# erlgo/openair4G

Measured on AMD Instinct MI355X. Metric: DL subframes/sec (20 MHz, 2x2, 64-QAM), higher is better.
Workload: dtype int16; 1 GPU; dlsim 20 MHz 2x2 TM3 (LARGE_CDD) 64-QAM MCS19x2CW, 2x14 IDFT-2048; config_id=C3, global_batch=8192, subframe_index=7, full_grid=False, parallelism=subframe-sharded x1

## Files before the change

### openair4g_amd/csrc/oai4g_encode.hip

```cpp
#include "oai4g_internal.h"

struct rsc_tables_t {
  uint8_t next[8][16];
  uint8_t par[8][16];
  uint8_t apow[8][8];
  uint32_t hz;
  uint32_t zs[8];
  uint32_t fm[3];
};

static constexpr uint8_t rsc_step_c(uint8_t u, uint8_t s, uint8_t *out)
{
  *out = (uint8_t)((u ^ (s >> 2) ^ (s >> 1)) & 1);
  return (uint8_t)((((u << 2) ^ (s >> 1)) ^ ((s >> 1) << 2) ^ (s << 2)) & 7);
}

static constexpr rsc_tables_t make_rsc_tables()
{
  rsc_tables_t t{};
  for (int s = 0; s < 8; s++)
    for (int nib = 0; nib < 16; nib++) {
      uint8_t st = (uint8_t)s, p = 0;
      for (int b = 0; b < 4; b++) {
        uint8_t o = 0;
// ... 90 lines not shown
typedef const __attribute__((address_space(1))) uint32_t gu32_t;

[[maybe_unused]] static __device__ __forceinline__ void gold_generate(uint32_t *gold, uint32_t nwords, uint32_t c_init,
                                                     const uint32_t *gx1, const uint32_t *gx2j)
{
  const uint32_t l = threadIdx.x, w0 = OAI4G_GOLD_STRIDE * l;
  if (l >= OAI4G_GOLD_LANES || w0 >= nwords) return;
  const uint32_t x2i = c_init ^ ((c_init ^ (c_init >> 1) ^ (c_init >> 2) ^ (c_init >> 3)) << 31);
  gu32_t *col = (gu32_t *)(gx2j + l);
  uint32_t cv[32];
#pragma unroll
  for (int b = 0; b < 32; b++) cv[b] = col[OAI4G_GOLD_LANES * b];
  uint32_t x2 = 0;
#pragma unroll
  for (int b = 0; b < 32; b++) x2 ^= cv[b] & (0u - ((x2i >> b) & 1u));
  uint32_t x1 = *(gu32_t *)(gx1 + l);
  const uint32_t wend = min(w0 + OAI4G_GOLD_STRIDE, nwords);
  gold[w0] = x1 ^ x2;
  for (uint32_t w = w0 + 1; w < wend; w++) {
    gold_step(x1, x2);
    gold[w] = x1 ^ x2;
  }
}

static __device__ __forceinline__ uint32_t crc_step(uint32_t reg, uint32_t byte, const uint32_t *tab)
{
  return ((reg << 8) & 0xffffffu) ^ tab[((reg >> 16) ^ byte) & 0xffu];
}

static __device__ __forceinline__ uint32_t crc_mul_tab(uint32_t a, const uint32_t *t )
{
  return t[a & 15u] ^ t[16 + ((a >> 4) & 15u)] ^ t[32 + ((a >> 8) & 15u)] ^ t[48 + ((a >> 12) & 15u)] ^
         t[64 + ((a >> 16) & 15u)] ^ t[80 + ((a >> 20) & 15u)];
}

static __device__ __forceinline__ uint32_t crc_chunk(const uint8_t *buf, uint32_t nbytes, uint32_t per, uint32_t lane,
                                                     uint32_t nl, const uint32_t *tab)
{
  const int vstart = (int)(lane * per) - (int)(per * nl - nbytes);
  uint32_t reg = 0;
  for (uint32_t i = 0; i < per; i += 4) {
    uint32_t b[4];
#pragma unroll
    for (int q = 0; q < 4; q++) {
      const int idx = vstart + (int)i + q;
      b[q] = idx >= 0 ? (uint32_t)buf[idx] : 0u;
    }
#pragma unroll
    for (int q = 0; q < 4; q++) reg = crc_step(reg, b[q], tab);
  }
  return reg;
}

static __device__ __forceinline__ uint32_t crc_chunk_w(const uint32_t *base32, uint32_t start, uint32_t nbytes,
                                                       uint32_t per, uint32_t lane, uint32_t nl, const uint32_t *tab8)
{
  const int vstart = (int)(lane * per) - (int)(per * nl - nbytes);
  uint32_t reg = 0;
  for (uint32_t i = 0; i < per; i += 4) {
    const int o = vstart + (int)i;
    const uint32_t a = start + (uint32_t)(o > 0 ? o : 0), wi = a >> 2;
    uint32_t w = __builtin_amdgcn_alignbit(base32[wi + 1], base32[wi], (a & 3u) * 8u);
    if (o < 0) w = o <= -4 ? 0u : w << (8 * (uint32_t)(-o));
    reg = (reg << 8) ^ tab8[(reg >> 24) ^ (w & 0xffu)];
    reg = (reg << 8) ^ tab8[(reg >> 24) ^ ((w >> 8) & 0xffu)];
    reg = (reg << 8) ^ tab8[(reg >> 24) ^ ((w >> 16) & 0xffu)];
    reg = (reg << 8) ^ tab8[(reg >> 24) ^ (w >> 24)];
  }
  return reg >> 8;
}

static __device__ __forceinline__ void crc_chunk_w2r(const uint32_t *base32, uint32_t start, uint32_t nbytes,
                                                     uint32_t per, uint32_t pos, uint32_t nl, const uint8_t *r2a,
                                                     const uint8_t *r2b, uint32_t &ra, uint32_t &rb)
{
  const int vstart = (int)(pos * per) - (int)(per * nl - nbytes);
  uint32_t a = 0, b = 0;
  for (uint32_t i = 0; i < per; i += 4) {
    const int o = vstart + (int)i;
    const uint32_t ad = start + (uint32_t)(o > 0 ? o : 0), wi = ad >> 2;
    uint32_t w = __builtin_amdgcn_alignbit(base32[wi + 1], base32[wi], (ad & 3u) * 8u);
    if (o < 0) w = o <= -4 ? 0u : w << (8 * (uint32_t)(-o));
    const uint32_t wr = __builtin_bitreverse32(w);
    const uint32_t x[4] = {wr >> 22, wr >> 14, wr >> 6, wr << 2};
#pragma unroll
    for (int q = 0; q < 4; q++) {
      a = (a >> 8) ^ *(const uint32_t *)(r2a + ((a ^ x[q]) & 0x3fcu));
      b = (b >> 8) ^ *(const uint32_t *)(r2b + ((b ^ x[q]) & 0x3fcu));
    }
  }
  ra = __builtin_bitreverse32(a >> 2) >> 8;
  rb = __builtin_bitreverse32(b >> 2) >> 8;
}

static __device__ __forceinline__ void crc_group_tree2(uint32_t &ra, uint32_t &rb, uint32_t pos, uint32_t lpb,
                                                       const uint32_t (*ma)[8][96], const uint32_t (*mb)[8][96])
{
  const uint32_t j0 = 7 - (pos & 7), j1 = (lpb >> 3) - 1 - (pos >> 3);
  ra = crc_mul_tab(ra, ma[0][j0]);
  rb = crc_mul_tab(rb, mb[0][j0]);
#pragma unroll
  for (int m = 1; m < 8; m <<= 1) {
    ra ^= __shfl_xor(ra, m, 64);
    rb ^= __shfl_xor(rb, m, 64);
  }
  ra = crc_mul_tab(ra, ma[1][j1]);
  rb = crc_mul_tab(rb, mb[1][j1]);
  for (uint32_t m = 8; m < lpb; m <<= 1) {
    ra ^= __shfl_xor(ra, (int)m, 64);
    rb ^= __shfl_xor(rb, (int)m, 64);
  }
}

[[maybe_unused]] static __device__ __forceinline__ uint32_t crc_wave_tree(uint32_t reg, const uint32_t *mul)
{
  const uint32_t lane = threadIdx.x & 63;
  for (int d = 0; d < 6; d++) {
    uint32_t other = __shfl_down(reg, 1u << d, 64);
    if ((lane & ((2u << d) - 1u)) == 0) reg = crc_mul_tab(reg, mul + d * 96) ^ other;
  }
  return reg;
}

static __device__ __forceinline__ uint32_t crc_wave_tree2(uint32_t reg, const uint32_t (*mul)[8][96])
{
  const uint32_t lane = threadIdx.x & 63;
  reg = crc_mul_tab(reg, mul[0][7 - (lane & 7)]);
  reg ^= __shfl_xor(reg, 1, 64);
  reg ^= __shfl_xor(reg, 2, 64);
  reg ^= __shfl_xor(reg, 4, 64);
  reg = crc_mul_tab(reg, mul[1][7 - (lane >> 3)]);
  reg ^= __shfl_xor(reg, 8, 64);
  reg ^= __shfl_xor(reg, 16, 64);
  reg ^= __shfl_xor(reg, 32, 64);
  return reg;
}

static __device__ __forceinline__ uint32_t crc_mulmod(uint32_t a, uint32_t b, uint32_t poly)
{
  uint32_t r = 0;
  for (int i = 23; i >= 0; i--) {
    r <<= 1;
    if (r & 0x1000000u) r ^= 0x1000000u | poly;
    if ((b >> i) & 1u) r ^= a;
  }
// ... 265 lines not shown
#pragma unroll
  for (int k = 0; k < 3; k++) {
    const uint32_t J = 4u >> k;
    const bool hi = (lane32 & J) != 0;
    t.rot[k] = hi ? J : 32u - J;
    t.mm[k] = hi ? ~M[k] : M[k];
  }
  return t;
}

template <int K = 0>
static __device__ __forceinline__ uint32_t transpose32_t(uint32_t x, const tp_lane_t &t)
{
  if constexpr (K == 5) {
    return x;
  } else if constexpr (K < 2) {
    const uint32_t p = xor_lane<(16u >> K)>(x);
    return transpose32_t<K + 1>(__builtin_amdgcn_perm(p, x, K == 0 ? t.sel16 : t.sel8), t);
  } else {
    const uint32_t p = xor_lane<(16u >> K)>(x);
    const uint32_t sh = __builtin_amdgcn_alignbit(p, p, t.rot[K - 2]);
    uint32_t r;
    asm("v_bitop3_b32 %0, %1, %2, %3 bitop3:0xe4" : "=v"(r) : "v"(x), "v"(sh), "v"(t.mm[K - 2]));
    return transpose32_t<K + 1>(r, t);
  }
}

static __device__ __forceinline__ void or_bits(uint32_t *w, uint32_t bit, uint32_t v)
{
  if (!v) return;
  const uint32_t wi = bit >> 5, sh = bit & 31u;
  atomicOr(&w[wi], v << sh);
  if (sh && (v >> (32 - sh))) atomicOr(&w[wi + 1], v >> (32 - sh));
}

static __device__ __forceinline__ void or_bits2(uint32_t *w, uint32_t bit, uint32_t v)
{
  const uint64_t s = (uint64_t)v << (bit & 31u);
  uint32_t *p = w + (bit >> 5);
  atomicOr(p, (uint32_t)s);
  atomicOr(p + 1, (uint32_t)(s >> 32));
}

template <bool DEBUG>
static __device__ void encode_codeword(const cfg_dev_t *__restrict__ c, uint32_t sf, uint32_t cwi,
                                       const uint8_t *__restrict__ payload, uint32_t *__restrict__ ebits,
                                       enc_debug_t dbg, uint32_t *lds_base, int stop_phase = 99, uint32_t sf0 = 0)
{
  const cw_dev_t &cw = c->cw[cwi];
  const uint32_t tid = threadIdx.x, nth = blockDim.x, lane = tid & 63, nwaves = nth >> 6;
  const uint32_t wave = __builtin_amdgcn_readfirstlane(tid >> 6);
  const uint32_t sfi = DEBUG ? sf : (c->first_sf + (sf0 + sf) * c->sf_step) % 10;
  const uint32_t C = __builtin_amdgcn_readfirstlane(cw.C), sw = __builtin_amdgcn_readfirstlane(cw.stream_words);
  uint32_t *tbw = lds_base;
  uint32_t *strm = lds_base + c->lds_a_words;
  uint32_t *crctab_a = strm;
  uint32_t *crctab_b = crctab_a + 256;
  uint32_t *tails = strm + c->lds_b_words;
  uint32_t *crcs = tails + 2 * OAI4G_MAX_CB;
  uint32_t *red = crcs + OAI4G_MAX_CB + 2;
  enc_tabs_t *tabs = (enc_tabs_t *)(red + 4);
  uint32_t *dbg_ebuf = (uint32_t *)(tabs + 1);
  uint8_t *tbb = (uint8_t *)tbw;
  const uint32_t G = cw.G[sfi];

  const uint32_t nw = cw.ilv_off[C], u0 = cw.u0, n0 = cw.n0;
  const uint32_t kw0 = __builtin_amdgcn_readfirstlane(cw.kw[0]), kw1 = __builtin_amdgcn_readfirstlane(cw.kw[1]);
  const uint32_t km0 = __builtin_amdgcn_readfirstlane(cw.kmag[0]), km1 = __builtin_amdgcn_readfirstlane(cw.kmag[1]);
  const uint32_t kk0 = __builtin_amdgcn_readfirstlane(cw.kk[0]), kk1 = __builtin_amdgcn_readfirstlane(cw.kk[1]);
  const uint32_t L8 = __builtin_amdgcn_readfirstlane(cw.L) >> 3, F8 = __builtin_amdgcn_readfirstlane(cw.F) >> 3;
  const uint32_t cb0 = (kk0 >> 3) - L8, cb1 = (kk1 >> 3) - L8;
  auto seg_of = [&](uint32_t r, uint32_t &fill, uint32_t &ncopy, uint32_t &s0) {
    const uint32_t ki = r >= n0 ? 1u : 0u;
    fill = r == 0 ? F8 : 0u;
    ncopy = (ki ? cb1 : cb0) - fill;
    s0 = r == 0 ? 0u : (ki ? n0 * cb0 + (r - n0) * cb1 : r * cb0) - F8;
  };

  const uint8_t *src = payload + (size_t)(DEBUG ? 0 : (sf * c->n_cw + cwi)) * c->payload_stride;
  const uint32_t Ab = cw.A_bytes;
  {
    const uint32_t ct = tid, cn = nth;
    for (uint32_t i = ct; i < c->lds_tb_words; i += cn) {
      uint32_t v = 0;
      if (4 * i < Ab) {
        v = *(const uint32_t *)(src + 4 * i);
        uint32_t valid = Ab - 4 * i;
        if (valid < 4) v &= (1u << (8 * valid)) - 1u;
      }
      tbw[i] = v;
    }
    if (ct == 0) crcs[0] = 0u;
    if (C > 1) {
      for (uint32_t v = ct; v < 256; v += cn) {
        const uint32_t iv = __builtin_bitreverse32(v) >> 24;
        crctab_a[v] = __builtin_bitreverse32(c->crctab[0][iv] << 8) << 2;
        crctab_b[v] = __builtin_bitreverse32(c->crctab[1][iv] << 8) << 2;
      }
    } else {
      for (uint32_t v = ct; v < 256; v += cn)
        crctab_a[v] = c->crctab[0][v] << 8;
    }
    for (uint32_t i = ct; i < 128; i += cn) {
      (&tabs->next[0][0])[i] = (&c_rsc.next[0][0])[i];
      (&tabs->par[0][0])[i] = (&c_rsc.par[0][0])[i];
      if (i < 64) (&tabs->apow[0][0])[i] = (&c_rsc.apow[0][0])[i];
      if (i < 8) tabs->zs[i] = c_rsc.zs[i];
    }
  }
  __syncthreads();
  if (stop_phase <= 0) return;

  if (C > 1) {
    const uint32_t lpb = __builtin_amdgcn_readfirstlane(cw.crc_lpb), per = __builtin_amdgcn_readfirstlane(cw.crc_per_cb);
    const uint32_t pos = tid & (lpb - 1);
    for (uint32_t r = tid / lpb; r < C; r += nth / lpb) {
      uint32_t fill, n, s0;
      seg_of(r, fill, n, s0);
      if (s0 + n > Ab) n = Ab > s0 ? Ab - s0 : 0;
      uint32_t ra, rb;
      crc_chunk_w2r(tbw, s0, n, per, pos, lpb, (const uint8_t *)crctab_a, (const uint8_t *)crctab_b, ra, rb);
      crc_group_tree2(ra, rb, pos, lpb, cw.crc2_cb[0], cw.crc2_cb[1]);
      if (pos == 0) {
        crcs[1 + r] = rb;
        atomicXor(&crcs[0], crc_mul_tab(ra, cw.crcmul_blk[r]));
      }
    }
    __syncthreads();
    if (tid == 0) {
      const uint32_t crc = crcs[0];
      tbb[Ab] = (uint8_t)(crc >> 16);
      tbb[Ab + 1] = (uint8_t)(crc >> 8);
      tbb[Ab + 2] = (uint8_t)crc;
      uint32_t a = __builtin_bitreverse32(crcs[C] << 8) << 2;
      const uint8_t *r2b = (const uint8_t *)crctab_b;
      a = (a >> 8) ^ *(const uint32_t *)(r2b + ((a ^ (__builtin_bitreverse32(crc >> 16) >> 22)) & 0x3fcu));
      a = (a >> 8) ^ *(const uint32_t *)(r2b + ((a ^ (__builtin_bitreverse32((crc >> 8) & 0xffu) >> 22)) & 0x3fcu));
      a = (a >> 8) ^ *(const uint32_t *)(r2b + ((a ^ (__builtin_bitreverse32(crc & 0xffu) >> 22)) & 0x3fcu));
      crcs[C] = __builtin_bitreverse32(a >> 2) >> 8;
    }
  } else {
    uint32_t reg = crc_chunk_w(tbw, 0, Ab, cw.crc_per_tb, tid, nth, crctab_a);
    reg = crc_wave_tree2(reg, cw.crc2_tb);
    if (lane == 0) red[wave] = reg;
    __syncthreads();
    if (tid == 0) {
      uint32_t v01 = crc_mul_tab(red[0], cw.crcmul_tb[6][0]) ^ red[1];
      uint32_t v23 = crc_mul_tab(red[2], cw.crcmul_tb[6][0]) ^ red[3];
      uint32_t crc = crc_mul_tab(v01, cw.crcmul_tb[7][0]) ^ v23;
      tbb[Ab] = (uint8_t)(crc >> 16);
      tbb[Ab + 1] = (uint8_t)(crc >> 8);
      tbb[Ab + 2] = (uint8_t)crc;
    }
  }
  __syncthreads();
  if (DEBUG && dbg.b)
    for (uint32_t i = tid; i < Ab + 3; i += nth) dbg.b[i] = tbb[i];
  if (stop_phase <= 1) return;

  for (uint32_t i = tid; i < C * 3 * 4; i += nth) {
    const uint32_t slot = i >> 2, r = slot / 3;
    const uint32_t w = (r < n0 ? kw0 : kw1) + (i & 3u);
    if (w < sw) strm[slot * sw + w] = 0u;
  }
  auto unit_of = [&](uint32_t i, uint32_t &r, uint32_t &j, uint32_t &K, uint32_t &ki) {
    ki = i >= u0 ? 1u : 0u;
    const uint32_t ii = ki ? i - u0 : i, kw = ki ? kw1 : kw0;
    const uint32_t rr = __umul24(ii, ki ? km1 : km0) >> 20;
    j = ii - __umul24(rr, kw);
    r = ki ? n0 + rr : rr;
    K = ki ? kk1 : kk0;
  };
  for (uint32_t i = tid; i < nw; i += nth) {
    uint32_t r, j, K, ki;
    unit_of(i, r, j, K, ki);
    uint32_t fill, ncopy, s0;
    seg_of(r, fill, ncopy, s0);
    const uint32_t i0 = 4 * j;
    uint32_t le;
    if (i0 >= fill) {
      const uint32_t a = s0 + i0 - fill, wi = a >> 2;
      le = __builtin_amdgcn_alignbit(tbw[wi + 1], tbw[wi], (a & 3u) * 8u);
      const int sh = (int)(fill + ncopy) - (int)i0;
      if (C > 1 && sh < 4) {
        const uint32_t crcle = __builtin_bswap32(crcs[1 + r] << 8);
        const uint32_t cw32 = (uint32_t)(((uint64_t)crcle << (8 * (sh + 4))) >> 32);
        le = (sh > 0 ? le & (0xffffffffu >> (32 - 8 * sh)) : 0u) | cw32;
      }
    } else {
      const uint32_t crcb = C > 1 ? crcs[1 + r] : 0;
      le = 0;
      for (uint32_t q = 0; q < 4; q++) {
        const uint32_t ib = i0 + q;
        uint32_t byte = 0;
        if (ib < fill) byte = 0;
        else if (ib < fill + ncopy) byte = tbb[s0 + ib - fill];
        else if (C > 1 && ib < fill + ncopy + 3) byte = (crcb >> (8 * (2 - (ib - fill - ncopy)))) & 0xffu;
        le |= byte << (8 * q);
      }
    }
    uint32_t wv = bytes_to_seq(le);
    if (32 * (j + 1) > K) wv &= (1u << (K - 32 * j)) - 1u;
    strm[r * 3 * sw + j] = wv;
  }
  __syncthreads();
  if (stop_phase <= 2) return;

  uint32_t *ilv = lds_base;
  const uint32_t fw0 = __builtin_amdgcn_readfirstlane(cw.qpp_f32[0]), fw1 = __builtin_amdgcn_readfirstlane(cw.qpp_f32[1]);
  const bool f32a = n0 != 0 && fw0 != 0, f32b = fw1 != 0;
  const uint32_t ft0 = f32a ? n0 * (kw0 >> 5) : 0u, ftn = ft0 + (f32b ? (C - n0) * (kw1 >> 5) : 0u);
  const uint32_t fm0 = fw0 >> 5, fm1 = fw1 >> 5;
  uint32_t *etab0 = strm + 2 * sw, *etab1 = strm + (n0 * 3 + 2) * sw;
  uint32_t te0 = 0, te1 = 0;
  if (f32a && tid < kw0) te0 = ((const uint16_t *)cw.qpp_tab[0])[tid];
  if (f32b && tid < kw1) te1 = ((const uint16_t *)cw.qpp_tab[1])[tid];
  auto tile_of = [&](uint32_t i, uint32_t &r, uint32_t &t, uint32_t &nt, uint32_t &ki) {
    ki = i >= ft0 ? 1u : 0u;
    const uint32_t ii = ki ? i - ft0 : i;
    nt = (ki ? kw1 : kw0) >> 5;
    const uint32_t rr = __umul24(ii, ki ? fm1 : fm0) >> 20;
    t = ii - __umul24(rr, nt);
    r = ki ? n0 + rr : rr;
  };
  if (ftn) {
    const tp_lane_t tpl = tp_lane(tid & 31);
    const uint32_t l32 = tid & 31u;
    const uint32_t sa = fw0 & 31u, sb = fw1 & 31u;
    for (uint32_t base = 0; base < ftn; base += nth >> 5) {
      uint32_t r, t, nt, ki;
      tile_of(min(base + (tid >> 5), ftn - 1), r, t, nt, ki);
      uint32_t *sys = strm + r * 3 * sw;
      const uint32_t v = sys[t + nt * (((ki ? sb : sa) * l32) & 31u)];
      sys[sw + 32 * t + l32] = transpose32_t<0>(v, tpl);
    }
    if (f32a && tid < kw0) etab0[tid] = te0;
    if (f32b && tid < kw1) etab1[tid] = te1;
  }
  for (uint32_t r = 0; r < C; r++) {
    if (r < n0 ? f32a : f32b) continue;
    const uint32_t K = r < n0 ? kk0 : kk1, Kw = (K + 31) >> 5, Q = K >> 2, io = r < n0 ? r * kw0 : u0 + (r - n0) * kw1;
    const uint32_t *sys = strm + r * 3 * sw;
    for (uint32_t w = tid; w < Kw; w += nth) ilv[io + w] = 0u;
    const uint32_t ng = (Q + 31) >> 5, nbw = (Q + 7) >> 3;
    for (uint32_t g = tid; g < ng; g += nth) {
      uint32_t P[4];
#pragma unroll
      for (uint32_t q = 0; q < 4; q++) {
        const uint32_t src = 32 * g + q * Q, wi = src >> 5;
        const uint32_t lo = sys[wi], hi = wi + 1 < Kw ? sys[wi + 1] : 0u;
        uint32_t v = __builtin_amdgcn_alignbit(hi, lo, src);
        if (src + 32 > K) v |= sys[0] << (K - src);
        P[q] = v;
      }
#pragma unroll
      for (uint32_t jb = 0; jb < 4; jb++) {
        const uint32_t t01 = __builtin_amdgcn_perm(P[1], P[0], 0x0c0c0000u | jb | ((4 + jb) << 8));
        const uint32_t t23 = __builtin_amdgcn_perm(P[3], P[2], 0x00000c0cu | (jb << 16) | ((4 + jb) << 24));
        if (4 * g + jb < nbw) strm[(r * 3 + 1) * sw + 4 * g + jb] = t01 | t23;
// ... 498 lines not shown
```

### openair4g_amd/csrc/oai4g_host.cpp

```cpp
#include <hip/hip_runtime.h>
#include <math.h>
#include <pthread.h>
#include <stdarg.h>
#include <stdio.h>
#include <stdlib.h>
#include <string.h>

#include <algorithm>
#include <cmath>
#include <cstdlib>
#include <vector>
#include <map>
#include <mutex>
#include <vector>

#include "../../include/oai4g.h"
#include "../../include/oai4g_qpp.h"
#include "../../include/oai4g_tbs.h"
#include "oai4g_internal.h"

static thread_local char g_err[512] = "";

static void set_err(const char *fmt, ...)
{
// ... 966 lines not shown
      c.t0k[ki] = (c.Rk[ki] + 31) / 32;
      c.ntk[ki] = c.t0k[ki] + (c.Rk[ki] + 15) / 16;
      c.ntmag[ki] = ((1u << 20) + c.ntk[ki] - 1) / c.ntk[ki];
      if (c.ntk[ki] > OAI4G_RM_TILES) { set_err("rate-matching plan: %u tiles", c.ntk[ki]); return -1; }
      rm_plan(c, ki);
    }
    if (oai4g_rm_pair_schedule(C, c.n0, c.ntk, c.rm_wrapt, c.rm_pairs, c.rm_pair0) < 0) {
      set_err("rate-matching pair schedule");
      return -1;
    }
    max_w = wwords > max_w ? wwords : max_w;
    uint32_t tbw = (c.A_bytes + 3 + 3) / 4 + 1;
    max_tb_words = tbw > max_tb_words ? tbw : max_tb_words;
    uint32_t strw = C * 3 * c.stream_words;
    max_stream_words = strw > max_stream_words ? strw : max_stream_words;
    for (int sf = 0; sf < 10; sf++) {
      int G;
      if (fp.nb_antennas_tx == 4) {
        std::vector<uint16_t> tmp((size_t)14 * fp.ofdm_symbol_size);
        uint32_t sb[14];
        int n = build_remap(&fp, p->rb_alloc, p->num_pdcch_symbols, sf, p->mimo_mode, tmp.data(), sb, nullptr);
        G = n < 0 ? -1 : n * (int)c.Qm;
      } else {
        G = oai4g_get_G(&fp, p->nb_rb, p->rb_alloc, (uint8_t)c.Qm, Nl[cw], p->num_pdcch_symbols, 0, (uint8_t)sf);
      }
      if (G <= 0 || G > OAI4G_MAX_CHANNEL_BITS) { set_err("G=%d out of range", G); return -1; }
      c.G[sf] = (uint32_t)G;
      uint32_t Gp = (uint32_t)G / Nl[cw] / c.Qm, GpmodC = Gp % C, off = 0;
      for (uint32_t r = 0; r < C; r++) {
        uint32_t E = (r < C - GpmodC) ? Nl[cw] * c.Qm * (Gp / C) : Nl[cw] * c.Qm * ((GpmodC ? 1 : 0) + Gp / C);
        c.E[sf][r] = E;
        c.roff[sf][r] = off;
        off += E;
      }
      c.roff[sf][C] = off;
      c.esplit[sf] = C - GpmodC;
      for (int h = 0; h < 2; h++) {
        const uint32_t E = c.E[sf][h ? C - 1 : 0], w = (E + 31) / 32;
        c.ew[sf][h] = w;
        c.emag[sf][h] = w ? (uint32_t)(((1ull << 32) + w - 1) / w) : 0u;
      }
      uint32_t gw = (off + 31) / 32;
      max_gw = gw > max_gw ? gw : max_gw;
      max_bits = (uint32_t)G > max_bits ? (uint32_t)G : max_bits;
    }
    qam_tables_scaled((int)c.Qm, p->amp, p->sqrt_rho_a, p->sqrt_rho_b, p->mimo_mode == OAI4G_ALAMOUTI, c);
  }
  if (max_gw > OAI4G_MAX_GOLD_WORDS) { set_err("G too large"); return -1; }
  h.lds_tb_words = max_tb_words;
  h.lds_stream_words = max_stream_words;
  h.lds_gold_words = max_gw + 1;
  h.lds_w_words = max_w;
  (void)max_inw;
  h.lds_a_words = max_tb_words;
  for (int cw = 0; cw < p->n_cw; cw++) {
    const cw_dev_t &c = h.cw[cw];
    if (c.ilv_off[c.C] > h.lds_a_words) h.lds_a_words = c.ilv_off[c.C];
    const uint32_t hb = (c.C + 1) / 2;
    for (int sf = 0; sf < 10; sf++) {
      const uint32_t G = c.G[sf], eb = hb < c.C ? c.roff[sf][hb] : G;
      const uint32_t w1 = (eb + 31) / 32 + 1, w2 = (G + 31) / 32 - eb / 32 + 1;
      if (w1 > h.lds_a_words) h.lds_a_words = w1;
      if (w2 > h.lds_a_words) h.lds_a_words = w2;
    }
  }
  h.lds_b_words = max_stream_words;
  if (h.lds_b_words < OAI4G_ENC_CRC_TABLE_WORDS) h.lds_b_words = OAI4G_ENC_CRC_TABLE_WORDS;

  if (need_remap) {
    uint32_t N = h.N;
    cfg->h_remap.assign((size_t)10 * 14 * N, 0xFFFF);
    for (int sf = 0; sf < 10; sf++) {
      if (only_sf >= 0 && sf != only_sf) continue;
      int n = build_remap(&fp, p->rb_alloc, p->num_pdcch_symbols, sf, p->mimo_mode,
                          cfg->h_remap.data() + (size_t)sf * 14 * N, h.symbase[sf], &cfg->re_alloc[sf]);
      if (n < 0) { set_err("RE map construction failed"); return -1; }
      cfg->re_count[sf] = n;
      if (p->with_crs) {
        uint32_t gt[20][2][14];
        lte_gold_table_h(&fp, gt);
        const uint32_t sps = fp.Ncp == 0 ? 7 : 6, psym[4] = {0, sps - 3, sps, 2 * sps - 3};
        const int nports = (fp.nb_antennas_tx > 1 && !fp.mode1_flag) ? 2 : 1;
        cfg->h_crs.resize((size_t)10 * 6 * 200);
        for (uint32_t i = 0; i < 4; i++) {
          const uint32_t Ns = 2 * sf + (i >> 1), l = i & 1;
          for (uint32_t m = 0; m < 2u * fp.N_RB_DL; m++) {
            const uint32_t mp = 110 - fp.N_RB_DL + m;
            cfg->h_crs[((size_t)sf * 6 + i) * 200 + m] = crs_qpsk(p->amp, (gt[Ns][l][mp >> 4] >> (2 * (mp & 15))) & 3);
            for (int port = 0; port < nports; port++) {
              uint16_t &code = cfg->h_remap[((size_t)sf * 14 + psym[i]) * N + crs_bin(&fp, port, l, m)];
              if (code != 0xFFFF) { set_err("CRS RE collides with a PDSCH RE"); return -1; }
              code = (uint16_t)(OAI4G_CRS_CODE | (i << 9) | ((uint32_t)port << 8) | m);
            }
          }
        }
        if (fp.nb_antennas_tx == 4)
          for (uint32_t s = 0; s < 2; s++) {
            const uint32_t Ns = 2 * sf + s;
            uint32_t gw[14];
            gold_words_h(&fp, Ns, 1, gw);
            for (uint32_t m = 0; m < 2u * fp.N_RB_DL; m++) {
              const uint32_t mp = 110 - fp.N_RB_DL + m;
              cfg->h_crs[((size_t)sf * 6 + 4 + s) * 200 + m] = crs_qpsk(p->amp, (gw[mp >> 4] >> (2 * (mp & 15))) & 3);
              for (uint32_t port = 2; port < 4; port++) {
                uint16_t &code = cfg->h_remap[((size_t)sf * 14 + s * sps + 1) * N + crs_bin_p23(&fp, port, Ns, m)];
                if (code != 0xFFFF) { set_err("CRS RE collides with a PDSCH RE"); return -1; }
                code = (uint16_t)(OAI4G_CRS_CODE | ((4 + s) << 9) | ((port & 1u) << 8) | m);
              }
            }
          }
      }
      h.pilmask = 0;
      for (uint32_t l = 0, hs = h.nsymb >> 1; l < h.nsymb; l++) {
        const uint32_t ls = l % hs;
        if (ls == 0 || ls == hs - 3 || (fp.nb_antennas_tx == 4 && ls == 1)) h.pilmask |= 1u << l;
      }
      for (int l = 0; l < 14; l++) {
        uint32_t next = l + 1 < (int)h.nsymb ? h.symbase[sf][l + 1] : (uint32_t)n;
        h.symnre[sf][l] = (uint32_t)(l < p->num_pdcch_symbols || l >= (int)h.nsymb ? 0 : next - h.symbase[sf][l]);
      }
// ... 3159 lines not shown
```

### openair4g_amd/csrc/oai4g_internal.h

```cpp
#pragma once
#include <hip/hip_runtime.h>
#include <stdint.h>

#include "../../include/oai4g.h"

#define OAI4G_MAX_CB 16
#define OAI4G_MAX_NULLS 104
#define OAI4G_MAX_CHUNKS 192
#define OAI4G_MAX_TASKS (OAI4G_MAX_CB * 20)
#define OAI4G_RM_TILES 20
#define OAI4G_RM_SRC_LAST (1u << 20)
#define OAI4G_RM_DST_WRAP (1u << 27)
#define OAI4G_PIPE_MAX_CHUNKS 16
#define OAI4G_CRS_CODE 0xE000u
#define OAI4G_CTL_CODE 0xC000u
static constexpr uint32_t oai4g_mod_entry_shift(uint32_t mimo_mode, uint32_t n_ant, uint32_t log2N)
{
  return log2N != 11 ? 1u : mimo_mode == OAI4G_LARGE_CDD && n_ant == 2 ? 3u : mimo_mode == OAI4G_SISO ? 2u : 1u;
}
static constexpr uint32_t oai4g_mod_addr_mask(uint32_t shift) { return 0x7FFFu & ~((1u << shift) - 1u); }
static constexpr uint32_t oai4g_mod_sentinel(uint32_t N) { return (3u * N) / 4u; }
static constexpr bool oai4g_mod_nre_fits(uint32_t nre, uint32_t N) { return nre + 3u <= oai4g_mod_sentinel(N); }
struct oai4g_mod_item_t {
  uint32_t sf, l, pair;
};
static constexpr uint32_t oai4g_mod_permag(uint32_t per) { return (uint32_t)(((1ull << 32) + per - 1) / per); }
static inline __host__ __device__ oai4g_mod_item_t oai4g_mod_item(uint32_t item, uint32_t ips, uint32_t lz, uint32_t per,
                                                                  uint32_t permag)
{
  const uint32_t it = item / ips;
  const uint32_t sf = (uint32_t)(((uint64_t)it * permag) >> 32);
  return {sf, lz + it - sf * per, item - it * ips};
}
#define OAI4G_MOD_LZ_MAX 4u
#define OAI4G_ENC_CRC_TABLE_WORDS (256 + 256)
#define OAI4G_GOLD_LANES 256
#define OAI4G_GOLD_STRIDE 17
#define OAI4G_MAX_GOLD_WORDS (OAI4G_GOLD_LANES * OAI4G_GOLD_STRIDE)
#define OAI4G_TW_TOTAL (16 + 64 + 128 + 256 + 512 + 1024 + 2048)

static inline __host__ __device__ uint32_t oai4g_tw_offset(int log2s)
{
  switch (log2s) {
  case 4: return 0;
  case 6: return 16;
  case 7: return 80;
  case 8: return 208;
  case 9: return 464;
  case 10: return 976;
  case 11: return 2000;
  default: return 0;
  }
}

struct cw_dev_t {
  uint32_t TBS;
  uint32_t A_bytes;
  uint32_t C, Cminus, Kplus, Kminus, F, L;
  uint32_t Qm;
  uint32_t q;
  uint32_t K[OAI4G_MAX_CB];
  uint32_t f1[OAI4G_MAX_CB], f2[OAI4G_MAX_CB];
  uint32_t src[OAI4G_MAX_CB];
  uint32_t fill[OAI4G_MAX_CB];
  uint32_t ncopy[OAI4G_MAX_CB];
  uint32_t crc_off[OAI4G_MAX_CB];
  uint32_t R[OAI4G_MAX_CB], Kpi[OAI4G_MAX_CB], ND[OAI4G_MAX_CB], Ncb[OAI4G_MAX_CB];
  uint32_t Nnn[OAI4G_MAX_CB];
  uint32_t k0c[OAI4G_MAX_CB];
  uint32_t kidx[OAI4G_MAX_CB];
  uint32_t wpk_off[OAI4G_MAX_CB + 1];
  uint32_t ntask;
  uint16_t tasks[OAI4G_MAX_TASKS];
  uint32_t ilv_off[OAI4G_MAX_CB + 1];
  uint32_t qpp0[2][OAI4G_MAX_CHUNKS];
  alignas(16) uint32_t qpp_tab[2][OAI4G_MAX_CHUNKS * 4];
  uint32_t qpp_f32[2];
  uint32_t qpp_s3[2];
  uint32_t n0, u0, kk[2], kw[2], kmag[2];
  uint32_t Rk[2], NDk[2], Ncbk[2], Nnnk[2], k0ck[2];
  uint32_t ntk[2], t0k[2], ntmag[2];
  uint32_t rm_wrapt[2];
  uint32_t nullcol[2][2];
  uint32_t esplit[10], ew[10][2], emag[10][2];
  uint32_t nnull[2];
  uint16_t nullpos[2][OAI4G_MAX_NULLS];
  uint32_t G[10];
  uint32_t E[10][OAI4G_MAX_CB];
  uint32_t roff[10][OAI4G_MAX_CB + 1];
  int16_t qam_a[8], qam_b[8];
  int16_t qpsk_a, qpsk_b;
  int16_t alm_qpsk[2][2];
// ... 267 lines not shown
```

### openair4g_amd/csrc/oai4g_ofdm.hip

```cpp
#include "oai4g_internal.h"

#include "oai4g_dft_prims.h"

__host__ __device__ constexpr int tw_distinct(int T, int SC, int J) { return T >= SC ? 1 : (SC / T < J ? SC / T : J); }

template <int LOG2N>
struct idft_tw_t {
  static constexpr int N = 1 << LOG2N, T = N >> 4;
  static constexpr bool HAS256 = LOG2N >= 8, HAS1024 = LOG2N >= 10, HASR2 = (LOG2N & 1) != 0;
  static constexpr int D64 = tw_distinct(T, 16, 4), D256 = tw_distinct(T, 64, 4), D1024 = tw_distinct(T, 256, 4),
                       DR2 = tw_distinct(T, N / 2, 8);
  twp_t l16[7];
  s16x2 l64[D64][3];
  s16x2 l256[HAS256 ? D256 : 1][3];
  s16x2 l1024[HAS1024 ? D1024 : 1][3];
  s16x2 r2[HASR2 ? DR2 : 1];

  __device__ __forceinline__ void load(const uint32_t *tw, int t)
  {
    gu32_t *g = (gu32_t *)tw;
    constexpr int i16[7] = {0, 1, 2, 3, 4, 6, 9};
#pragma unroll
    for (int i = 0; i < 7; i++)
      l16[i] = {u2c(g[oai4g_tw_offset(4) + i16[i]]), u2c(g[OAI4G_TW_TOTAL + oai4g_tw_offset(4) + i16[i]])};
// ... 599 lines not shown
static __device__ __forceinline__ s16x2 alm_ta(uint32_t bits, const cw_dev_t &w, uint32_t pil)
{
  if (w.Qm == 2) {
    const short p = w.alm_qpsk[pil][0], n = w.alm_qpsk[pil][1];
    return (s16x2){(bits & 1) ? n : p, (bits & 2) ? n : p};
  }
  return qam_map(bits, w.Qm, pil ? w.qam_b : w.qam_a, 0);
}
static __device__ __forceinline__ s16x2 alm_tb(uint32_t bits, const cw_dev_t &w, uint32_t pil)
{
  if (w.Qm == 2) {
    const short p = w.alm_qpsk[pil][0], n = w.alm_qpsk[pil][1];
    return (s16x2){(bits & 1) ? p : n, (bits & 2) ? n : p};
  }
  const s16x2 v = qam_map(bits, w.Qm, pil ? w.qam_b : w.qam_a, 0);
  return (s16x2){(short)-v.x, v.y};
}
static __device__ __forceinline__ void alm_pair(s16x2 ta, s16x2 tb, uint32_t role, s16x2 &y0, s16x2 &y1)
{
  y0 = role ? (s16x2){(short)-tb.x, tb.y} : ta;
  y1 = role ? (s16x2){ta.x, (short)-ta.y} : tb;
}

__host__ __device__ constexpr uint32_t cdd4_mask(bool neg)
{
  constexpr int8_t M4[4][4][2] = {{{1, 1}, {1, 1}, {1, -1}, {-1, 1}},
                                  {{1, -1}, {1, 1}, {-1, 1}, {1, 1}},
                                  {{1, 1}, {-1, 1}, {1, 1}, {1, -1}},
                                  {{1, -1}, {-1, 1}, {-1, -1}, {-1, -1}}};
  uint32_t m = 0;
  for (int i8 = 0; i8 < 8; i8++)
    for (int p = 0; p < 4; p++) {
      const int a = M4[i8 >> 1][p][0], b = M4[i8 >> 1][p][1] * ((i8 & 1) ? -1 : 1);
      if (neg ? a < 0 : a != b) m |= 1u << (i8 * 4 + p);
    }
  return m;
}
static constexpr uint32_t CDD4_QSEL = cdd4_mask(false), CDD4_NEG = cdd4_mask(true);

static __device__ __forceinline__ s16x2 half_signed(s16x2 x, bool neg)
{
  const s16x2 h = x >> (s16x2){1, 1};
  const s16x2 nh = u2c(~c2u(h)) + u2c(~c2u(x) & 0x00010001u);
  return neg ? nh : h;
}

template <int LOG2N>
struct modofdm_geom {
  static constexpr int N = 1 << LOG2N, T = N >> 4, UNITS = 128 / T, LDSW = idft_sel<LOG2N>::XW;
  static constexpr int SENT = oai4g_mod_sentinel(N), SW = SENT + 4, QPT = 3, QROW = 64;
  static constexpr int ZLO = LOG2N == 8 ? 6 : 5, ZHI = LOG2N == 8 ? 9 : 10;
};
static constexpr bool modofdm_zband(int MODE, bool CRS) { return CRS || MODE != 2; }

typedef uint32_t __attribute__((aligned(1))) u32_a1_t;
static __device__ __forceinline__ uint32_t ld_u32_any(const uint8_t *p)
{
  return *(const __attribute__((address_space(1))) u32_a1_t *)p;
}

#define MODOFDM_WAVES_OF(L) (OAI4G_MODOFDM_WAVES > 0 ? OAI4G_MODOFDM_WAVES : ((L) == 11 ? 4 : 3))
#define MODOFDM_ATTR __attribute__((amdgpu_waves_per_eu(MODOFDM_WAVES_OF(LOG2N))))
template <int LOG2N, int MODE, bool CRS, bool ECP, bool NS = false>
__global__ void __launch_bounds__(128) MODOFDM_ATTR k_modofdm(const cfg_dev_t *__restrict__ c, int n_items,
                                                 const uint32_t *__restrict__ ebits, int32_t *__restrict__ iq,
                                                 uint32_t sf0)
{
  using G = modofdm_geom<LOG2N>;
  constexpr int N = G::N, T = G::T, UNITS = G::UNITS, LDSW = G::LDSW;
  constexpr int NA = MODE == 0 ? 1 : 2;
  constexpr bool CW2 = MODE == 2 || MODE == 3;
  constexpr uint32_t IPS = MODE == 3 ? 2u : 1u;
  __shared__ __attribute__((aligned(16))) uint32_t lds_data[UNITS * NA * LDSW];
  constexpr bool SEARLY = CRS && (NA == 1 || LOG2N < 11);
  constexpr int SW = G::SW, SENT = G::SENT, QPT = G::QPT, QROW = G::QROW;
  constexpr uint32_t QZERO = 4u * 4u * QROW;
  constexpr bool ALIAS = LOG2N == 11;
  static_assert(!ALIAS || (UNITS == 1 && 2 * SW <= 2 * NA * LDSW), "staged addresses must fit the exchange");
  __shared__ __attribute__((aligned(16))) uint16_t lds_s_own[ALIAS ? 1 : UNITS][2][SW];
  uint16_t(*lds_s)[2][SW] = ALIAS ? (uint16_t(*)[2][SW])lds_data : lds_s_own;
  __shared__ uint32_t qtab[4 * QROW + 1];
  constexpr uint32_t ESH = oai4g_mod_entry_shift(MODE == 0 ? OAI4G_SISO : MODE == 1 ? OAI4G_ALAMOUTI : OAI4G_LARGE_CDD,
                                                 MODE == 3 ? 4 : 2, LOG2N);
  constexpr uint32_t EMASK = oai4g_mod_addr_mask(ESH);
  constexpr bool PRE = ESH == 3;
  static_assert(!PRE || (MODE == 2 && ALIAS && SW * 8 <= NA * LDSW * 4), "the precoded pairs must fit the exchange");
  u32x2_t *lds_p = (u32x2_t *)lds_data;
  constexpr bool PRE1 = ESH == 2;
  static_assert(!PRE1 || (MODE == 0 && ALIAS && SW * 4 <= NA * LDSW * 4), "the staged QAM words must fit the exchange");
  uint32_t *lds_w = (uint32_t *)lds_data;
  const int unit = threadIdx.x / T, t = threadIdx.x % T;
  typename idft_sel<LOG2N>::tw_t twr;
  twr.load(c->tw, t);
  const uint32_t n_ant = c->n_ant;
  constexpr uint32_t sps = ECP ? 6 : 7;
  for (uint32_t i = threadIdx.x; i < 4 * QROW + 1; i += blockDim.x) {
    const uint32_t row = i / QROW, bits = i - row * QROW, cw = row >> 1, pil = row & 1;
    uint32_t v = 0;
    if (row < 4) {
      if constexpr (MODE == 1) {
        const cw_dev_t &w = c->cw[0];
        v = c2u(cw ? alm_tb(bits, w, pil) : alm_ta(bits, w, pil));
      } else {
        const cw_dev_t &w = c->cw[cw];
        v = c2u(qam_map(bits, w.Qm, pil ? w.qam_b : w.qam_a, pil ? w.qpsk_b : w.qpsk_a));
      }
    }
    qtab[i] = v;
  }
  if (!ALIAS)
    for (uint32_t i = threadIdx.x; i < UNITS * 4; i += blockDim.x) lds_s[i >> 2][(i >> 1) & 1][SENT + (i & 1)] = QZERO;
  const uint32_t Qm0 = c->cw[0].Qm, Qm1 = c->cw[1].Qm;
// ... 500 lines not shown
```

Measured before the change: 9.173 million subframes/s.

## Load transport block directly into per-code-block stream layout, computing CRCs in place

The transport-block payload is no longer staged in an LDS byte buffer and then re-segmented into code-block stream words. Instead each wave loads payload words straight from global memory into the bit-reversed systematic stream slots, handling filler and tail masking inline. CRCs are computed over the stream layout using bit-reversed tables and written into the stream tail bytes, which removes a separate segmentation pass and a barrier. The CRC tables move to the LDS region formerly used by the TB buffer, shrinking LDS use. The price is more complex masking logic and unaligned global loads, and CRC bytes are now inserted by byte stores after the fact.

```diff
diff --git a/openair4g_amd/csrc/oai4g_encode.hip b/openair4g_amd/csrc/oai4g_encode.hip
--- a/openair4g_amd/csrc/oai4g_encode.hip
+++ b/openair4g_amd/csrc/oai4g_encode.hip
@@ -166,22 +166,12 @@
   return reg;
 }
 
-static __device__ __forceinline__ uint32_t crc_chunk_w(const uint32_t *base32, uint32_t start, uint32_t nbytes,
-                                                       uint32_t per, uint32_t lane, uint32_t nl, const uint32_t *tab8)
-{
-  const int vstart = (int)(lane * per) - (int)(per * nl - nbytes);
-  uint32_t reg = 0;
-  for (uint32_t i = 0; i < per; i += 4) {
-    const int o = vstart + (int)i;
-    const uint32_t a = start + (uint32_t)(o > 0 ? o : 0), wi = a >> 2;
-    uint32_t w = __builtin_amdgcn_alignbit(base32[wi + 1], base32[wi], (a & 3u) * 8u);
-    if (o < 0) w = o <= -4 ? 0u : w << (8 * (uint32_t)(-o));
-    reg = (reg << 8) ^ tab8[(reg >> 24) ^ (w & 0xffu)];
-    reg = (reg << 8) ^ tab8[(reg >> 24) ^ ((w >> 8) & 0xffu)];
-    reg = (reg << 8) ^ tab8[(reg >> 24) ^ ((w >> 16) & 0xffu)];
-    reg = (reg << 8) ^ tab8[(reg >> 24) ^ (w >> 24)];
-  }
-  return reg >> 8;
+static __device__ __forceinline__ uint32_t crc_stream_word(const uint32_t *base32, uint32_t start, int o)
+{
+  const uint32_t ad = start + (uint32_t)(o > 0 ? o : 0), wi = ad >> 2;
+  uint32_t w = __builtin_amdgcn_alignbit(base32[wi + 1], base32[wi], (ad & 3u) * 8u);
+  if (o < 0) w = o <= -4 ? 0u : w << (8 * (uint32_t)(-o));
+  return w;
 }
 
 static __device__ __forceinline__ void crc_chunk_w2r(const uint32_t *base32, uint32_t start, uint32_t nbytes,
@@ -191,12 +181,8 @@
   const int vstart = (int)(pos * per) - (int)(per * nl - nbytes);
   uint32_t a = 0, b = 0;
   for (uint32_t i = 0; i < per; i += 4) {
-    const int o = vstart + (int)i;
-    const uint32_t ad = start + (uint32_t)(o > 0 ? o : 0), wi = ad >> 2;
-    uint32_t w = __builtin_amdgcn_alignbit(base32[wi + 1], base32[wi], (ad & 3u) * 8u);
-    if (o < 0) w = o <= -4 ? 0u : w << (8 * (uint32_t)(-o));
-    const uint32_t wr = __builtin_bitreverse32(w);
-    const uint32_t x[4] = {wr >> 22, wr >> 14, wr >> 6, wr << 2};
+    const uint32_t w = crc_stream_word(base32, start, vstart + (int)i);
+    const uint32_t x[4] = {w << 2, w >> 6, w >> 14, w >> 22};
 #pragma unroll
     for (int q = 0; q < 4; q++) {
       a = (a >> 8) ^ *(const uint32_t *)(r2a + ((a ^ x[q]) & 0x3fcu));
@@ -205,6 +191,25 @@
   }
   ra = __builtin_bitreverse32(a >> 2) >> 8;
   rb = __builtin_bitreverse32(b >> 2) >> 8;
+}
+
+static __device__ __forceinline__ uint32_t crc_chunk_w1r(const uint32_t *base32, uint32_t start, uint32_t nbytes,
+                                                         uint32_t per, uint32_t pos, uint32_t nl, const uint8_t *r2a)
+{
+  const int vstart = (int)(pos * per) - (int)(per * nl - nbytes);
+  uint32_t a = 0;
+  for (uint32_t i = 0; i < per; i += 4) {
+    const uint32_t w = crc_stream_word(base32, start, vstart + (int)i);
+    const uint32_t x[4] = {w << 2, w >> 6, w >> 14, w >> 22};
+#pragma unroll
+    for (int q = 0; q < 4; q++) a = (a >> 8) ^ *(const uint32_t *)(r2a + ((a ^ x[q]) & 0x3fcu));
+  }
+  return __builtin_bitreverse32(a >> 2) >> 8;
+}
+
+static __device__ __forceinline__ uint32_t crc_step_r2(uint32_t a, uint32_t byte, const uint8_t *r2)
+{
+  return (a >> 8) ^ *(const uint32_t *)(r2 + ((a ^ (__builtin_bitreverse32(byte) >> 22)) & 0x3fcu));
 }
 
 static __device__ __forceinline__ void crc_group_tree2(uint32_t &ra, uint32_t &rb, uint32_t pos, uint32_t lpb,
@@ -576,16 +581,14 @@
   const uint32_t wave = __builtin_amdgcn_readfirstlane(tid >> 6);
   const uint32_t sfi = DEBUG ? sf : (c->first_sf + (sf0 + sf) * c->sf_step) % 10;
   const uint32_t C = __builtin_amdgcn_readfirstlane(cw.C), sw = __builtin_amdgcn_readfirstlane(cw.stream_words);
-  uint32_t *tbw = lds_base;
   uint32_t *strm = lds_base + c->lds_a_words;
-  uint32_t *crctab_a = strm;
+  uint32_t *crctab_a = lds_base;
   uint32_t *crctab_b = crctab_a + 256;
   uint32_t *tails = strm + c->lds_b_words;
   uint32_t *crcs = tails + 2 * OAI4G_MAX_CB;
   uint32_t *red = crcs + OAI4G_MAX_CB + 2;
   enc_tabs_t *tabs = (enc_tabs_t *)(red + 4);
   uint32_t *dbg_ebuf = (uint32_t *)(tabs + 1);
-  uint8_t *tbb = (uint8_t *)tbw;
   const uint32_t G = cw.G[sfi];
 
   const uint32_t nw = cw.ilv_off[C], u0 = cw.u0, n0 = cw.n0;
@@ -604,32 +607,69 @@
   const uint8_t *src = payload + (size_t)(DEBUG ? 0 : (sf * c->n_cw + cwi)) * c->payload_stride;
   const uint32_t Ab = cw.A_bytes;
   {
-    const uint32_t ct = tid, cn = nth;
-    for (uint32_t i = ct; i < c->lds_tb_words; i += cn) {
-      uint32_t v = 0;
-      if (4 * i < Ab) {
-        v = *(const uint32_t *)(src + 4 * i);
-        uint32_t valid = Ab - 4 * i;
-        if (valid < 4) v &= (1u << (8 * valid)) - 1u;
-      }
-      tbw[i] = v;
-    }
-    if (ct == 0) crcs[0] = 0u;
-    if (C > 1) {
-      for (uint32_t v = ct; v < 256; v += cn) {
-        const uint32_t iv = __builtin_bitreverse32(v) >> 24;
-        crctab_a[v] = __builtin_bitreverse32(c->crctab[0][iv] << 8) << 2;
-        crctab_b[v] = __builtin_bitreverse32(c->crctab[1][iv] << 8) << 2;
-      }
-    } else {
-      for (uint32_t v = ct; v < 256; v += cn)
-        crctab_a[v] = c->crctab[0][v] << 8;
-    }
-    for (uint32_t i = ct; i < 128; i += cn) {
-      (&tabs->next[0][0])[i] = (&c_rsc.next[0][0])[i];
-      (&tabs->par[0][0])[i] = (&c_rsc.par[0][0])[i];
-      if (i < 64) (&tabs->apow[0][0])[i] = (&c_rsc.apow[0][0])[i];
-      if (i < 8) tabs->zs[i] = c_rsc.zs[i];
+    constexpr uint32_t ENC_BLK = 6;
+    const uint32_t nsl = (kw1 + 63) >> 6;
+    const uint32_t lim = ((Ab + 3) & ~3u) - 4;
+    for (uint32_t sl = wave; sl < nsl; sl += nwaves) {
+      const uint32_t j0 = sl << 6, j = j0 + lane, i0 = 4 * j;
+      for (uint32_t rb = 0; rb < C; rb += ENC_BLK) {
+        uint32_t v[ENC_BLK];
+#pragma unroll
+        for (uint32_t u = 0; u < ENC_BLK; u++) {
+          const uint32_t r = rb + u;
+          v[u] = 0;
+          if (r >= C) break;
+          uint32_t fill, ncopy, s0;
+          seg_of(r, fill, ncopy, s0);
+          const uint32_t a = s0 + (i0 > fill ? i0 - fill : 0u);
+          v[u] = ld_u32_any(src + min(a, lim));
+        }
+#pragma unroll
+        for (uint32_t u = 0; u < ENC_BLK; u++) {
+          const uint32_t r = rb + u;
+          if (r >= C) break;
+          const uint32_t kw = r < n0 ? kw0 : kw1;
+          if (j0 >= kw) continue;
+          uint32_t fill, ncopy, s0;
+          seg_of(r, fill, ncopy, s0);
+          const uint32_t nd = s0 + ncopy > Ab ? (Ab > s0 ? Ab - s0 : 0u) : ncopy;
+          const uint32_t dend = fill + nd;
+          uint32_t *sys = strm + r * 3 * sw;
+          if ((sl == 0 && fill != 0) || 4 * (j0 + 64) > dend) {
+            if (j < kw) {
+              const int pre = (int)fill - (int)i0, valid = (int)dend - (int)i0;
+              const uint32_t a = s0 + (pre < 0 ? (uint32_t)-pre : 0u);
+              uint32_t le = v[u] >> ((8 * (a - min(a, lim))) & 31u);
+              if (pre > 0) le <<= (8 * (uint32_t)pre) & 31u;
+              if (valid < 4) le &= (1u << ((8 * (uint32_t)valid) & 31u)) - 1u;
+              if (valid <= 0 || pre >= 4) le = 0;
+              sys[j] = bytes_to_seq(le);
+            }
+          } else {
+            sys[j] = bytes_to_seq(v[u]);
+          }
+        }
+      }
+    }
+    for (uint32_t i = tid; i < C * 3 * 4; i += nth) {
+      const uint32_t slot = i >> 2, r = slot / 3;
+      const uint32_t w = (r < n0 ? kw0 : kw1) + (i & 3u);
+      if (w < sw) strm[slot * sw + w] = 0u;
+    }
+    if (tid == 0) crcs[0] = 0u;
+    {
+      const uint32_t tv = __builtin_bitreverse32(tid) >> 24, tr = tid & 127u;
+      const uint32_t ta = c->crctab[0][tv], tb = c->crctab[1][tv];
+      const uint32_t rsc_n = (&c_rsc.next[0][0])[tr], rsc_p = (&c_rsc.par[0][0])[tr];
+      const uint32_t rsc_a = (&c_rsc.apow[0][0])[tr & 63u], rsc_z = c_rsc.zs[tr & 7u];
+      crctab_a[tid] = __builtin_bitreverse32(ta << 8) << 2;
+      if (C > 1) crctab_b[tid] = __builtin_bitreverse32(tb << 8) << 2;
+      if (tid < 128) {
+        (&tabs->next[0][0])[tid] = (uint8_t)rsc_n;
+        (&tabs->par[0][0])[tid] = (uint8_t)rsc_p;
+        if (tid < 64) (&tabs->apow[0][0])[tid] = (uint8_t)rsc_a;
+        if (tid < 8) tabs->zs[tid] = rsc_z;
+      }
     }
   }
   __syncthreads();
@@ -643,7 +683,8 @@
       seg_of(r, fill, n, s0);
       if (s0 + n > Ab) n = Ab > s0 ? Ab - s0 : 0;
       uint32_t ra, rb;
-      crc_chunk_w2r(tbw, s0, n, per, pos, lpb, (const uint8_t *)crctab_a, (const uint8_t *)crctab_b, ra, rb);
+      crc_chunk_w2r(strm, 4 * (r * 3 * sw) + fill, n, per, pos, lpb, (const uint8_t *)crctab_a, (const uint8_t *)crctab_b, ra,
+                    rb);
       crc_group_tree2(ra, rb, pos, lpb, cw.crc2_cb[0], cw.crc2_cb[1]);
       if (pos == 0) {
         crcs[1 + r] = rb;
@@ -651,42 +692,53 @@
       }
     }
     __syncthreads();
+    if (tid >= 1 && tid < C) {
+      const uint32_t r = tid - 1;
+      const uint32_t v = __builtin_bitreverse32(crcs[1 + r] << 8);
+      uint8_t *p = (uint8_t *)(strm + r * 3 * sw) + ((r < n0 ? kk0 : kk1) >> 3) - 3;
+      p[0] = (uint8_t)v;
+      p[1] = (uint8_t)(v >> 8);
+      p[2] = (uint8_t)(v >> 16);
+    }
     if (tid == 0) {
       const uint32_t crc = crcs[0];
-      tbb[Ab] = (uint8_t)(crc >> 16);
-      tbb[Ab + 1] = (uint8_t)(crc >> 8);
-      tbb[Ab + 2] = (uint8_t)crc;
       uint32_t a = __builtin_bitreverse32(crcs[C] << 8) << 2;
       const uint8_t *r2b = (const uint8_t *)crctab_b;
-      a = (a >> 8) ^ *(const uint32_t *)(r2b + ((a ^ (__builtin_bitreverse32(crc >> 16) >> 22)) & 0x3fcu));
-      a = (a >> 8) ^ *(const uint32_t *)(r2b + ((a ^ (__builtin_bitreverse32((crc >> 8) & 0xffu) >> 22)) & 0x3fcu));
-      a = (a >> 8) ^ *(const uint32_t *)(r2b + ((a ^ (__builtin_bitreverse32(crc & 0xffu) >> 22)) & 0x3fcu));
-      crcs[C] = __builtin_bitreverse32(a >> 2) >> 8;
+      a = crc_step_r2(a, crc >> 16, r2b);
+      a = crc_step_r2(a, (crc >> 8) & 0xffu, r2b);
+      a = crc_step_r2(a, crc & 0xffu, r2b);
+      const uint32_t va = __builtin_bitreverse32(crc << 8), vb = a >> 2;
+      uint8_t *p = (uint8_t *)(strm + (C - 1) * 3 * sw) + (kk1 >> 3) - 6;
+      p[0] = (uint8_t)va;
+      p[1] = (uint8_t)(va >> 8);
+      p[2] = (uint8_t)(va >> 16);
+      p[3] = (uint8_t)vb;
+      p[4] = (uint8_t)(vb >> 8);
+      p[5] = (uint8_t)(vb >> 16);
     }
   } else {
-    uint32_t reg = crc_chunk_w(tbw, 0, Ab, cw.crc_per_tb, tid, nth, crctab_a);
-    reg = crc_wave_tree2(reg, cw.crc2_tb);
+    const uint32_t reg = crc_wave_tree2(crc_chunk_w1r(strm, F8, Ab, cw.crc_per_tb, tid, nth, (const uint8_t *)crctab_a), cw.crc2_tb);
     if (lane == 0) red[wave] = reg;
     __syncthreads();
     if (tid == 0) {
       uint32_t v01 = crc_mul_tab(red[0], cw.crcmul_tb[6][0]) ^ red[1];
       uint32_t v23 = crc_mul_tab(red[2], cw.crcmul_tb[6][0]) ^ red[3];
       uint32_t crc = crc_mul_tab(v01, cw.crcmul_tb[7][0]) ^ v23;
-      tbb[Ab] = (uint8_t)(crc >> 16);
-      tbb[Ab + 1] = (uint8_t)(crc >> 8);
-      tbb[Ab + 2] = (uint8_t)crc;
-    }
-  }
-  __syncthreads();
-  if (DEBUG && dbg.b)
-    for (uint32_t i = tid; i < Ab + 3; i += nth) dbg.b[i] = tbb[i];
-  if (stop_phase <= 1) return;
-
-  for (uint32_t i = tid; i < C * 3 * 4; i += nth) {
-    const uint32_t slot = i >> 2, r = slot / 3;
-    const uint32_t w = (r < n0 ? kw0 : kw1) + (i & 3u);
-    if (w < sw) strm[slot * sw + w] = 0u;
-  }
+      const uint32_t va = __builtin_bitreverse32(crc << 8);
+      uint8_t *p = (uint8_t *)strm + F8 + Ab;
+      p[0] = (uint8_t)va;
+      p[1] = (uint8_t)(va >> 8);
+      p[2] = (uint8_t)(va >> 16);
+      if (DEBUG) crcs[0] = crc;
+    }
+  }
+  __syncthreads();
+  if (DEBUG && dbg.b) {
+    for (uint32_t i = tid; i < Ab; i += nth) dbg.b[i] = src[i];
+    if (tid < 3) dbg.b[Ab + tid] = (uint8_t)(crcs[0] >> (8 * (2 - tid)));
+  }
+  if (stop_phase <= 2) return;
+
   auto unit_of = [&](uint32_t i, uint32_t &r, uint32_t &j, uint32_t &K, uint32_t &ki) {
     ki = i >= u0 ? 1u : 0u;
     const uint32_t ii = ki ? i - u0 : i, kw = ki ? kw1 : kw0;
@@ -695,40 +747,6 @@
     r = ki ? n0 + rr : rr;
     K = ki ? kk1 : kk0;
   };
-  for (uint32_t i = tid; i < nw; i += nth) {
-    uint32_t r, j, K, ki;
-    unit_of(i, r, j, K, ki);
-    uint32_t fill, ncopy, s0;
-    seg_of(r, fill, ncopy, s0);
-    const uint32_t i0 = 4 * j;
-    uint32_t le;
-    if (i0 >= fill) {
-      const uint32_t a = s0 + i0 - fill, wi = a >> 2;
-      le = __builtin_amdgcn_alignbit(tbw[wi + 1], tbw[wi], (a & 3u) * 8u);
-      const int sh = (int)(fill + ncopy) - (int)i0;
-      if (C > 1 && sh < 4) {
-        const uint32_t crcle = __builtin_bswap32(crcs[1 + r] << 8);
-        const uint32_t cw32 = (uint32_t)(((uint64_t)crcle << (8 * (sh + 4))) >> 32);
-        le = (sh > 0 ? le & (0xffffffffu >> (32 - 8 * sh)) : 0u) | cw32;
-      }
-    } else {
-      const uint32_t crcb = C > 1 ? crcs[1 + r] : 0;
-      le = 0;
-      for (uint32_t q = 0; q < 4; q++) {
-        const uint32_t ib = i0 + q;
-        uint32_t byte = 0;
-        if (ib < fill) byte = 0;
-        else if (ib < fill + ncopy) byte = tbb[s0 + ib - fill];
-        else if (C > 1 && ib < fill + ncopy + 3) byte = (crcb >> (8 * (2 - (ib - fill - ncopy)))) & 0xffu;
-        le |= byte << (8 * q);
-      }
-    }
-    uint32_t wv = bytes_to_seq(le);
-    if (32 * (j + 1) > K) wv &= (1u << (K - 32 * j)) - 1u;
-    strm[r * 3 * sw + j] = wv;
-  }
-  __syncthreads();
-  if (stop_phase <= 2) return;
 
   uint32_t *ilv = lds_base;
   const uint32_t fw0 = __builtin_amdgcn_readfirstlane(cw.qpp_f32[0]), fw1 = __builtin_amdgcn_readfirstlane(cw.qpp_f32[1]);
diff --git a/openair4g_amd/csrc/oai4g_host.cpp b/openair4g_amd/csrc/oai4g_host.cpp
--- a/openair4g_amd/csrc/oai4g_host.cpp
+++ b/openair4g_amd/csrc/oai4g_host.cpp
@@ -1042,7 +1042,7 @@
   h.lds_gold_words = max_gw + 1;
   h.lds_w_words = max_w;
   (void)max_inw;
-  h.lds_a_words = max_tb_words;
+  h.lds_a_words = OAI4G_ENC_CRC_TABLE_WORDS;
   for (int cw = 0; cw < p->n_cw; cw++) {
     const cw_dev_t &c = h.cw[cw];
     if (c.ilv_off[c.C] > h.lds_a_words) h.lds_a_words = c.ilv_off[c.C];
@@ -1055,7 +1055,6 @@
     }
   }
   h.lds_b_words = max_stream_words;
-  if (h.lds_b_words < OAI4G_ENC_CRC_TABLE_WORDS) h.lds_b_words = OAI4G_ENC_CRC_TABLE_WORDS;
 
   if (need_remap) {
     uint32_t N = h.N;
diff --git a/openair4g_amd/csrc/oai4g_internal.h b/openair4g_amd/csrc/oai4g_internal.h
--- a/openair4g_amd/csrc/oai4g_internal.h
+++ b/openair4g_amd/csrc/oai4g_internal.h
@@ -38,6 +38,12 @@
 #define OAI4G_GOLD_STRIDE 17
 #define OAI4G_MAX_GOLD_WORDS (OAI4G_GOLD_LANES * OAI4G_GOLD_STRIDE)
 #define OAI4G_TW_TOTAL (16 + 64 + 128 + 256 + 512 + 1024 + 2048)
+
+typedef uint32_t __attribute__((aligned(1))) u32_a1_t;
+static __device__ __forceinline__ uint32_t ld_u32_any(const uint8_t *p)
+{
+  return *(const __attribute__((address_space(1))) u32_a1_t *)p;
+}
 
 static inline __host__ __device__ uint32_t oai4g_tw_offset(int log2s)
 {
diff --git a/openair4g_amd/csrc/oai4g_ofdm.hip b/openair4g_amd/csrc/oai4g_ofdm.hip
--- a/openair4g_amd/csrc/oai4g_ofdm.hip
+++ b/openair4g_amd/csrc/oai4g_ofdm.hip
@@ -675,12 +675,6 @@
   static constexpr int ZLO = LOG2N == 8 ? 6 : 5, ZHI = LOG2N == 8 ? 9 : 10;
 };
 static constexpr bool modofdm_zband(int MODE, bool CRS) { return CRS || MODE != 2; }
-
-typedef uint32_t __attribute__((aligned(1))) u32_a1_t;
-static __device__ __forceinline__ uint32_t ld_u32_any(const uint8_t *p)
-{
-  return *(const __attribute__((address_space(1))) u32_a1_t *)p;
-}
 
 #define MODOFDM_WAVES_OF(L) (OAI4G_MODOFDM_WAVES > 0 ? OAI4G_MODOFDM_WAVES : ((L) == 11 ? 4 : 3))
 #define MODOFDM_ATTR __attribute__((amdgpu_waves_per_eu(MODOFDM_WAVES_OF(LOG2N))))
```

Measured after the change: 9.441 million subframes/s, median of 6. +2.9%, better.
